# RustAudio/lewton

Measured on AMD Instinct MI355X. Metric: audio packets/sec (44.1 kHz stereo, 2048-pt long blocks), higher is better.
Workload: dtype f32; 1 GPU; BASELINE configs[1]: batches of 4096 synthetic 44.1 kHz stereo long-block (n=2048) packets per GPU = 256 streams x 16 consecutive packets, 8 batches rotated, records resident in HBM; streams_per_batch=256, channels=2, blocksize=2048, output=i16 planar, kernels=k_long, parity=unchecked (bench.py --full checks the timed batch against the oracle), parallelism=streams sharded across GPUs, no collectives

## Files before the change

lewton_amd/build.py:

```python
import os
import subprocess
import sys

HERE = os.path.dirname(os.path.abspath(__file__))
CSRC = os.path.join(HERE, "csrc")
LIBDIR = os.path.join(HERE, "_lib")
LIB = os.path.join(LIBDIR, "liblewton_amd.so")
SOURCES = ["lw_headers.cpp", "lw_entropy.cpp", "lw_dev_entropy.cpp", "lw_pool.cpp", "lw_runtime.cpp", "lw_batch.cpp", "lw_packet.cpp", "lw_fast.cpp", "lw_ring.cpp", "lw_shard.cpp", "lw_ogg.cpp", "lw_rows.cpp", "lw_rows_mix.cpp", "lw_capi.cpp", "lw_kernels.hip", "lw_kernels_long.hip", "lw_kernels_big.hip", "lw_kernels_entropy.hip", "lw_kernels_rows.hip", "lw_kernels_rows_mix.hip"]
ARCH = os.environ.get("LW_OFFLOAD_ARCH", "gfx950")
FLAGS = ["--offload-arch=" + ARCH, "-O3", "-std=c++17", "-ffp-contract=off", "-fno-fast-math", "-fPIC", "-Wall",
         "-Wno-unused-result", "-pthread"]


PER_FILE_FLAGS = {"lw_kernels_long.hip": ["-fno-slp-vectorize"]}


def hipcc():
    for c in (os.environ.get("HIPCC"), "/opt/rocm/bin/hipcc", "hipcc"):
        if c and (os.path.isabs(c) and os.path.exists(c) or not os.path.isabs(c)):
            return c
    raise RuntimeError("hipcc not found")


def needs_build():
    if not os.path.exists(LIB):
        return True
    t = os.path.getmtime(LIB)
    for root in (CSRC, os.path.join(HERE, "..", "include")):
        for f in os.listdir(root):
            if os.path.getmtime(os.path.join(root, f)) > t:
                return True
    return False


def build(force=False, verbose=False):
    if not force and not needs_build():
        return LIB
# ... 28 lines not shown
```

lewton_amd/csrc/lw_fast.hpp:

```cpp
#pragma once

#include "lw_host.hpp"
#include "lw_records.h"

#include <cstdint>
#include <vector>

#define LW_FAST_BS 11
#define LW_FAST_MAX_FLOORS 2
#define LW_FLOOR_EXACT_ADX 4096u
#define LW_FAST_WAVES 16
#define LW_FAST_MAX_ROUNDS 16

struct LwFastImage {
	uint32_t apair;
	uint32_t tw_s2;
	uint32_t tw_l0;
	uint32_t tw_l1;
	uint32_t tw_l2;
	uint32_t tw_l3;
	uint32_t tw_l4;
	uint32_t a2;
	uint32_t c4;
	uint32_t b_lo;
// ... 92 lines not shown
	LwFastImage off;
	const uint8_t *d_image;
	const LwFastItem *d_items;
	uint32_t n_items;
	const LwFastItem *d_halo_items;
	uint32_t n_halo_items;
	uint32_t n_units;
	uint32_t per_round;
	uint32_t rounds;
	uint32_t dense;
	uint32_t late_from;
	uint32_t has_tdonly;
	uint32_t split;
	uint32_t edge_mode;
	float *d_edge;
	uint32_t edge_n;
	const uint16_t *d_sid12;
	LwFastUnit units[LW_FAST_WAVES];
	float *d_halo;
	uint32_t pre_on;
	uint32_t pre[LW_FAST_WAVES];
};

#define LW_BLK_MIN_BS 8
#define LW_BLK_MAX_BS 10
#define LW_BLK_MAX_SLOTS 8
#define LW_BIG_MIN_BS 12
#define LW_BIG_MAX_BS 13
#define LW_BIG_MAX_PASSES 64u
#define LW_BLK_MAX_POSTS(L) ((L) >= 16 ? 64 : 32)

template <int L>
struct LwBlkLayout {
	static constexpr uint32_t APAIR = 0;
	static constexpr uint32_t TW_S2 = APAIR + 64u * L;
	static constexpr uint32_t TW_L0 = TW_S2 + 32u * L;
	static constexpr uint32_t TW_L1 = TW_L0 + 16u * L;
	static constexpr uint32_t TW_C2 = TW_L1 + 8u * L;
	static constexpr uint32_t TW_C3 = TW_C2 + 128u;
	static constexpr uint32_t A2 = TW_C3 + 64u;
	static constexpr uint32_t C4 = A2 + 16u;
	static constexpr uint32_t B_LO = C4 + 32u * L;
	static constexpr uint32_t B_HI = B_LO + 32u * L;
	static constexpr uint32_t WIN = B_HI + 32u * L;
	static constexpr uint32_t INV_DB = WIN + 64u * L;
	static constexpr uint32_t XSF = INV_DB + 1024u;
// ... 99 lines not shown
```

lewton_amd/csrc/lw_kernels_long.hip:

```cpp
#include <algorithm>
#include <cstddef>
#include <mutex>

#include "lw_fast.hpp"
#include "lw_kernels.hpp"
#include "lw_pcm_store.inc"

#define LW_WG (64 * LW_FAST_WAVES)
#define LW_PRIO_FLOOR 2
#define LW_PRIO_IMDCT 0
#define LW_PRIO_FINISH 3
#define LW_FLOOR_FIRST_FROM 7
#define LW_IMDCT_PRIO_LATE 12
#define LW_PRIO_PACE 0
#define LW_PRIO_READY 3
#define LW_SCR_BYTES 4096u
#define LW_PUB_BYTES 4096u
#define LW_LDS_BYTES (LWI_TOTAL + LW_FAST_WAVES * (LW_SCR_BYTES + LW_PUB_BYTES) + 3 * LW_FAST_WAVES * 4)

#include "lw_stamps.inc"

struct LwFastArgs {
	const float *residue;
	const uint16_t *floors;
	uint32_t n_items;
	uint32_t n_units;
	uint32_t per_round;
	uint32_t rounds;
	uint32_t dense;
	uint32_t late_from;
	uint32_t ch, fstride;
	LwFastUnit waves[LW_FAST_WAVES];
	const uint8_t *image;
	const LwFastItem *items;
	float *state;
	float *td;
	float *halo;
	float *edge;
	void *out;
	uint32_t state_stride, state_chan_stride;
	uint32_t edge_n;
// ... 249 lines not shown
	    "v_cndmask_b32_e64 %10, %5, -%5, %14\n\tv_cndmask_b32_e64 %11, %7, -%7, %15\n\t"
	    "v_add_f32_e32 %8, %0, %8\n\tv_add_f32_e32 %9, %2, %9\n\tv_add_f32_e32 %10, %4, %10\n\tv_add_f32_e32 %11, %6, %11\n\t"
	    "v_cndmask_b32_e64 %1, %0, %8, %16\n\tv_cndmask_b32_e64 %3, %2, %9, %17\n\t"
	    "v_cndmask_b32_e64 %5, %4, %10, %18\n\tv_cndmask_b32_e64 %7, %6, %11, %19\n\t"
	    "v_cndmask_b32_e64 %0, %8, %0, %16\n\tv_cndmask_b32_e64 %2, %9, %2, %17\n\t"
	    "v_cndmask_b32_e64 %4, %10, %4, %18\n\tv_cndmask_b32_e64 %6, %11, %6, %19"
	    : "+v"(m0), "+v"(a0), "+v"(m1), "+v"(a1), "+v"(m2), "+v"(a2), "+v"(m3), "+v"(a3), "=&v"(t0), "=&v"(t1), "=&v"(t2), "=&v"(t3),
	      "=&s"(c0), "=&s"(c1), "=&s"(c2), "=&s"(c3), "=&s"(d0), "=&s"(d1), "=&s"(d2), "=&s"(d3));
}

struct ItemRegs {
	uint32_t res_off, floor_off, out_off, src_arg;
	int32_t state_out;
	uint32_t halo_out, src_kind, flags;
	uint32_t pkt;
};

struct Pref {
	float4_t r[2][4];
	uint32_t fe[2];
};


__device__ __forceinline__ void issue_floor_loads(const LwFastArgs &F, const ItemRegs &it, const LwFastUnit &un, uint32_t lane,
		Pref &p)
{
	const uint16_t *f0 = F.floors + it.floor_off + (uint32_t)un.ch_a * F.fstride;
	p.fe[0] = lane < un.F_a ? (uint32_t)f0[lane] : 0u;
	p.fe[1] = 0u;
	if (un.ch_b >= 0) {
		const uint16_t *f1 = F.floors + it.floor_off + (uint32_t)un.ch_b * F.fstride;
		p.fe[1] = lane < un.F_b ? (uint32_t)f1[lane] : 0u;
	}
}

template <bool PAIR = false, bool NT = true>
__device__ __forceinline__ void issue_residue_loads(const LwFastArgs &F, const ItemRegs &it, const LwFastUnit &un,
		uint32_t lane, Pref &p)
{
	const float4_t *s0 = reinterpret_cast<const float4_t *>(F.residue + it.res_off + (uint32_t)un.ch_a * 1024u);
#pragma unroll
	for (int x = 0; x < 4; x++)
		p.r[0][x] = NT ? __builtin_nontemporal_load(&s0[64 * x + lane]) : s0[64 * x + lane];
	if (PAIR || un.ch_b >= 0) {
		const float4_t *s1 = reinterpret_cast<const float4_t *>(F.residue + it.res_off + (uint32_t)un.ch_b * 1024u);
#pragma unroll
		for (int x = 0; x < 4; x++)
			p.r[1][x] = NT ? __builtin_nontemporal_load(&s1[64 * x + lane]) : s1[64 * x + lane];
	}
}

template <bool NT = true>
__device__ __forceinline__ void issue_loads(const LwFastArgs &F, const ItemRegs &it, const LwFastUnit &un, uint32_t lane, Pref &p)
{
	issue_residue_loads<false, NT>(F, it, un, lane, p);
	issue_floor_loads(F, it, un, lane, p);
}

struct PreRegs {
	float4_t t[2][4];
};

__device__ __forceinline__ void issue_pre_loads(const LwFastArgs &F, const ItemRegs &it, uint32_t prog, uint32_t lane, PreRegs &q)
{
#pragma unroll
	for (int k = 0; k < 2; k++) {
		const uint32_t c = (prog >> (8 * k)) & 0xffu;
		if (c != LW_PRE_NO_CH) {
			const float4_t *s = reinterpret_cast<const float4_t *>(F.residue + it.res_off + c * 1024u);
#pragma unroll
			for (int x = 0; x < 4; x++)
				q.t[k][x] = s[64 * x + lane];
		} else {
#pragma unroll
			for (int x = 0; x < 4; x++)
				asm volatile("" : "=v"(q.t[k][x]));
		}
	}
}

#define LW_FLOOR_W0 2097153.0f
#define LW_FLOOR_MASK 0x7fcu
__device__ __forceinline__ bool floor_table(const LwFastArgs &F, const char *img, char *sc, uint32_t lane, uint32_t e,
		uint32_t fslot, uint32_t Fp)
{
	const bool unused = __builtin_amdgcn_readfirstlane(e) == LW_FLOOR_UNUSED;
// ... 473 lines not shown
#pragma nounroll
		for (uint32_t i = 0; i < n; i++) {
			switch ((prog >> (16u + 4u * i)) & 0xfu) {
			case 0x1: couple_quad(v0, v1); break;
			case 0x2: couple_quad(v0, v2); break;
			case 0x3: couple_quad(v0, v3); break;
			case 0x4: couple_quad(v1, v0); break;
			case 0x6: couple_quad(v1, v2); break;
			case 0x7: couple_quad(v1, v3); break;
			case 0x8: couple_quad(v2, v0); break;
			case 0x9: couple_quad(v2, v1); break;
			case 0xb: couple_quad(v2, v3); break;
			case 0xc: couple_quad(v3, v0); break;
			case 0xd: couple_quad(v3, v1); break;
			case 0xe: couple_quad(v3, v2); break;
			default: break;
			}
		}
		pf.r[0][x] = v0;
		pf.r[1][x] = v1;
	}
}

template <int NCH, bool SPLIT = false>
__device__ __forceinline__ void spectrum_fused(const LwFastArgs &F, const char *img, char *sc, uint32_t lane,
		const LwFastUnit &un, Pref &pf)
{
	__builtin_amdgcn_s_setprio(LW_PRIO_FLOOR);
	const bool unused0 = floor_table(F, img, sc, lane, pf.fe[0], un.floor_a, un.F_a);
	bool unused1 = false;
	if (NCH == 2)
		unused1 = floor_table(F, img, sc + 1024, lane, pf.fe[1], un.floor_b, un.F_b);
	lds_fence();
	if (NCH == 2 && un.coupled)
		decouple_pair(pf);
	if (SPLIT && NCH == 1 && un.coupled >= LW_UNIT_SPLIT_MAG) {
		if (un.coupled == LW_UNIT_SPLIT_ANG) {
#pragma unroll
			for (int x = 0; x < 4; x++) {
				const float4_t t = pf.r[0][x];
				pf.r[0][x] = pf.r[1][x];
				pf.r[1][x] = t;
			}
			decouple_pair(pf);
#pragma unroll
			for (int x = 0; x < 4; x++)
				pf.r[0][x] = pf.r[1][x];
		} else {
			decouple_pair(pf);
		}
	}
// ... 331 lines not shown
	}
}

typedef uint32_t u32x8_t __attribute__((ext_vector_type(8)));

__device__ __forceinline__ ItemRegs load_item(const LwFastItem *items, uint32_t idx)
{
	const LwFastItem *p = items + __builtin_amdgcn_readfirstlane(idx);
	u32x8_t v;
	asm volatile("s_load_dwordx8 %0, %1, 0x0\n\ts_waitcnt lgkmcnt(0)" : "=s"(v) : "s"(p) : "memory");
	ItemRegs it;
	it.res_off = v[0];
	it.floor_off = v[1];
	it.out_off = v[2];
	it.src_arg = v[3];
	it.state_out = (int32_t)v[4];
	it.halo_out = v[5];
	it.src_kind = v[6] & 0xffu;
	it.flags = (v[6] >> 16) & 0xffu;
	it.pkt = v[7];
	return it;
}

__device__ __forceinline__ void dense_offsets(const LwFastArgs &F, uint32_t item, ItemRegs &it)
{
	it.res_off = item * F.ch * 1024u;
	it.floor_off = item * F.ch * F.fstride;
}

#define LW_CNT_BASE (LWI_TOTAL + LW_FAST_WAVES * (LW_SCR_BYTES + LW_PUB_BYTES))
#define LW_CNT_PUB(w) (LW_CNT_BASE + 4u * (w))
#define LW_CNT_ACK(w) (LW_CNT_BASE + 4u * (LW_FAST_WAVES + (w)))
#define LW_CNT_LANDED(w) (LW_CNT_BASE + 4u * (2 * LW_FAST_WAVES + (w)))

__device__ __forceinline__ uint32_t lds_load_u32(uint32_t byte_addr)
{
	uint32_t v;
	asm volatile("ds_read_b32 %0, %1\n\ts_waitcnt lgkmcnt(0)" : "=v"(v) : "v"(byte_addr) : "memory");
	return v;
}

__device__ __forceinline__ void lds_store_u32(uint32_t byte_addr, uint32_t v)
{
	asm volatile("ds_write_b32 %0, %1" ::"v"(byte_addr), "v"(v) : "memory");
}

__device__ __forceinline__ void lds_wait_ge(uint32_t byte_addr, uint32_t need)
{
	while (__builtin_amdgcn_readfirstlane(lds_load_u32(byte_addr)) < need)
		__builtin_amdgcn_s_sleep(1);
}

template <int FMT, bool RIGHT_ONLY, bool TD = false, bool EDGE = false, bool SPLIT = false, bool PRE = false>
__global__ void __launch_bounds__(LW_WG) k_long(LwFastArgs F)
{
	constexpr bool MIXF = false, mix_drop_flags = false;
	uint32_t *const edge_flags = nullptr;
#include "lw_long_body.inc"
}

#define LW_SHORT_SPLIT_BELOW 1024u

template <int L>
struct LwBlkLds {
	static constexpr uint32_t SLOTS = 64u / L;
	static constexpr uint32_t POSTS = LW_BLK_MAX_POSTS(L);
	static constexpr uint32_t PT = POSTS / L;
};

template <int L, bool ONE = false>
struct LwBlkWave {
	static constexpr uint32_t SLOTS = 64u / L, POSTS = LW_BLK_MAX_POSTS(L), CH = ONE ? 1u : 2u;
	static constexpr uint32_t SCR = 0;
	static constexpr uint32_t PUB = 4096u;
	static constexpr uint32_t PUB_PASS = SLOTS * CH * 2u * L * 16u;
	static constexpr uint32_t REC = PUB + (ONE ? 1u : 2u) * PUB_PASS;
	static constexpr uint32_t TAB = REC + SLOTS * CH * POSTS * 2u;
	static constexpr uint32_t BYTES = TAB + SLOTS * CH * POSTS * 16u;
};
static_assert(LwBlkWave<8>::PUB_PASS == 4096u && LwBlkWave<32>::PUB_PASS == 4096u, "right parts of one pass: 4 KB");

// ... 304 lines not shown
	const uint32_t i = wave - (LW_FAST_WAVES - LW_MIX_SHORT_WAVES);
	const uint32_t wid = blockIdx.x * LW_MIX_SHORT_WAVES + i;
	if (wid >= F.n_waves)
		return;
	char *const smem_all = smem_dyn + LW_MIX_IMG_OFF;
	char *const smem = smem_dyn + LWI_TOTAL + (i < 2u ? 0u : LW_FAST_WAVES * LW_SCR_BYTES) + LW_MIX_LONG_WAVES * LW_SCR_BYTES +
		(i & 1u) * LwBlkWave<L, true>::BYTES;
	constexpr bool STAGE = false;
	if (__builtin_amdgcn_readfirstlane((uint32_t)F.units[wid % F.n_units].slot) == 0u) {
		constexpr int ONLY = 0;
#include "lw_short_body.inc"
	} else {
		constexpr int ONLY = 1;
#include "lw_short_body.inc"
	}
}

template <int FMT>
__global__ void __launch_bounds__(LW_WG) k_mix(LwFastArgs F, LwShortArgs FS, LwMixArgs M)
{
	constexpr bool RIGHT_ONLY = false, TD = false, EDGE = true, SPLIT = true, MIXF = true, PRE = false;
	uint32_t *const edge_flags = M.flags;
	const bool mix_drop_flags = M.drop_flags != 0;
#define LW_LONG_BODY_AFTER_STAGE                                                  \
	if (wave >= LW_FAST_WAVES - LW_MIX_SHORT_WAVES) {                            \
		mix_short_role<FMT>(FS, M, smem, wave, lane_id);                          \
		return;                                                                   \
	}
	static_assert(LwBlkLayout<8>::TOTAL / 16u <= 256u + 64u, "one 16-byte row per thread of four waves, a second one for the first 64");
#define LW_LONG_BODY_STAGE_LOAD                                                                       \
	const bool s_on = t >= 512u, s_two = s_on && t - 512u < LwBlkLayout<8>::TOTAL / 16u - 256u;       \
	const uint4 *s_src = reinterpret_cast<const uint4 *>(FS.image) + (s_on ? t - 512u : 0u);          \
	uint4 s_v0 = make_uint4(0, 0, 0, 0), s_v1 = s_v0;                                                 \
	if (s_on)                                                                                         \
		s_v0 = s_src[0];                                                                              \
	if (s_two)                                                                                        \
		s_v1 = s_src[256];
#define LW_LONG_BODY_STAGE_STORE                                                                      \
	uint4 *s_dst = reinterpret_cast<uint4 *>(smem + LW_MIX_IMG_OFF) + (s_on ? t - 512u : 0u);         \
	if (s_on)                                                                                         \
		s_dst[0] = s_v0;                                                                              \
	if (s_two)                                                                                        \
		s_dst[256] = s_v1;
#include "lw_long_body.inc"
#undef LW_LONG_BODY_AFTER_STAGE
#undef LW_LONG_BODY_STAGE_LOAD
#undef LW_LONG_BODY_STAGE_STORE
}

template <int L>
static hipError_t launch_short(LwShortArgs &F, int fmt, hipStream_t st)
{
	const dim3 grid(F.n_waves), block(64);
	return lw_with_out_fmt(fmt, [&](auto f) { return lw_launch_k(k_short<f.value, L>, grid, block, 0, st, F); });
}

static void short_prepare(const LwDevTables &T, const LwBatchDev &B, const LwShortLaunch &L, void *out, LwShortArgs &F)
{
	F.residue = B.residue;
	F.floors = B.floors;
	F.slots = L.d_slots;
	F.image = L.d_image;
	F.state = B.state;
	F.td = B.td;
	F.edge = L.d_edge;
	F.out = out;
	F.ch = T.ch;
// ... 29 lines not shown
	if (L.lanes == 16)
		return launch_short<16>(F, fmt, st);
	if (L.lanes == 32)
		return launch_short<32>(F, fmt, st);
	return hipErrorInvalidValue;
}

static hipError_t long_prepare(const LwDevTables &T, const LwBatchDev &B, const LwFastLaunch &L, void *out, hipStream_t st, LwFastArgs &F,
		uint32_t &grid)
{
	F.image = L.d_image;
	F.residue = B.residue;
	F.floors = B.floors;
	F.state = B.state;
	F.td = B.td;
	F.ch = T.ch;
	F.fstride = T.fstride;
	F.state_stride = T.state_stride;
	F.state_chan_stride = T.state_chan_stride;
	F.n_units = L.n_units;
	F.halo = L.d_halo;
	F.edge = L.d_edge;
	F.out = out;
	const size_t lds = LW_LDS_BYTES + LW_STAMP_LDS_EXTRA;
	for (uint32_t w = 0; w < LW_FAST_WAVES; w++) {
		F.waves[w] = L.units[w % L.n_units];
		F.waves[w].slot = (uint8_t)(w / L.n_units);
		F.pre[w] = L.pre_on ? L.pre[w % L.n_units] : 0u;
	}
	F.late_from = 0xFFFFFFFFu;
	static LwPerDeviceOnce once;
	const hipError_t attr_err = once.run([] {
		const void *fns[] = {(const void *)k_long<LW_OUT_I16_PLANAR, false>, (const void *)k_long<LW_OUT_I16_INTERLEAVED, false>,
			(const void *)k_long<LW_OUT_I16_ITL_STEREO, false>, (const void *)k_long<LW_OUT_F32_PLANAR, false>,
			(const void *)k_long<LW_OUT_I16_PLANAR, true>, (const void *)k_long<LW_OUT_I16_PLANAR, false, true>,
			(const void *)k_long<LW_OUT_I16_INTERLEAVED, false, true>, (const void *)k_long<LW_OUT_I16_ITL_STEREO, false, true>,
			(const void *)k_long<LW_OUT_F32_PLANAR, false, true>, (const void *)k_long<LW_OUT_I16_PLANAR, false, false, true>,
			(const void *)k_long<LW_OUT_I16_INTERLEAVED, false, false, true>, (const void *)k_long<LW_OUT_F32_PLANAR, false, false, true>,
			(const void *)k_long<LW_OUT_I16_PLANAR, true, false, false, true>,
			(const void *)k_long<LW_OUT_I16_PLANAR, false, false, false, true>, (const void *)k_long<LW_OUT_I16_INTERLEAVED, false, false, false, true>,
			(const void *)k_long<LW_OUT_F32_PLANAR, false, false, false, true>, (const void *)k_long<LW_OUT_I16_PLANAR, false, false, true, true>,
			(const void *)k_long<LW_OUT_I16_INTERLEAVED, false, false, true, true>, (const void *)k_long<LW_OUT_F32_PLANAR, false, false, true, true>,
			(const void *)k_mix<LW_OUT_I16_PLANAR>, (const void *)k_mix<LW_OUT_I16_INTERLEAVED>, (const void *)k_mix<LW_OUT_F32_PLANAR>,
			(const void *)k_long<LW_OUT_I16_PLANAR, true, false, false, false, true>,
			(const void *)k_long<LW_OUT_I16_PLANAR, false, false, false, false, true>, (const void *)k_long<LW_OUT_I16_INTERLEAVED, false, false, false, false, true>,
			(const void *)k_long<LW_OUT_F32_PLANAR, false, false, false, false, true>,
			(const void *)k_long<LW_OUT_I16_PLANAR, false, true, false, false, true>, (const void *)k_long<LW_OUT_I16_INTERLEAVED, false, true, false, false, true>,
// ... 2 lines not shown
			(const void *)k_long<LW_OUT_F32_PLANAR, false, false, true, false, true>,
			(const void *)k_long<LW_OUT_F32_ITL_STEREO, false>, (const void *)k_long<LW_OUT_F32_ITL_STEREO, false, true>,
			(const void *)k_long<LW_OUT_F32_INTERLEAVED, false>, (const void *)k_long<LW_OUT_F32_INTERLEAVED, false, true>,
			(const void *)k_long<LW_OUT_F32_INTERLEAVED, false, false, true>, (const void *)k_long<LW_OUT_F32_INTERLEAVED, false, false, false, true>,
			(const void *)k_long<LW_OUT_F32_INTERLEAVED, false, false, true, true>,
			(const void *)k_long<LW_OUT_F32_INTERLEAVED, false, false, false, false, true>,
			(const void *)k_long<LW_OUT_F32_INTERLEAVED, false, true, false, false, true>,
			(const void *)k_long<LW_OUT_F32_INTERLEAVED, false, false, true, false, true>, (const void *)k_mix<LW_OUT_F32_INTERLEAVED>};
		for (const void *f : fns) {
			const hipError_t e = hipFuncSetAttribute(f, hipFuncAttributeMaxDynamicSharedMemorySize, 160 * 1024);
			if (e != hipSuccess)
				return e;
		}
		return hipSuccess;
	});
	if (attr_err != hipSuccess)
		return attr_err;
	if (L.n_halo_items) {
		F.items = L.d_halo_items;
		F.n_items = L.n_halo_items;
		F.per_round = 1;
		F.rounds = 1;
		const hipError_t e = L.pre_on
			? lw_launch_k(k_long<LW_OUT_I16_PLANAR, true, false, false, false, true>, dim3(L.n_halo_items), dim3(LW_WG), lds, st, F)
			: L.split
			? lw_launch_k(k_long<LW_OUT_I16_PLANAR, true, false, false, true>, dim3(L.n_halo_items), dim3(LW_WG), lds, st, F)
			: lw_launch_k(k_long<LW_OUT_I16_PLANAR, true>, dim3(L.n_halo_items), dim3(LW_WG), lds, st, F);
		if (e != hipSuccess)
			return e;
	}
	grid = 0;
	if (L.n_items) {
		F.items = L.d_items;
		F.n_items = L.n_items;
		F.per_round = L.per_round;
		F.rounds = L.rounds;
		F.dense = L.dense;
		const uint32_t chunk = L.per_round * L.rounds;
		grid = (L.n_items + chunk - 1) / chunk;
		F.late_from = L.late_from;
	}
	return hipSuccess;
}

template <int FMT>
static hipError_t launch_long_main(const LwFastLaunch &L, LwFastArgs &F, uint32_t grid, size_t lds, hipStream_t st)
{
	constexpr int FP = lw_out_unit_free(FMT);
	if (L.pre_on) {
		if (L.edge_mode)
			return lw_launch_k(k_long<FP, false, false, true, false, true>, dim3(grid), dim3(LW_WG), lds, st, F);
		if (L.has_tdonly)
			return lw_launch_k(k_long<FP, false, true, false, false, true>, dim3(grid), dim3(LW_WG), lds, st, F);
		return lw_launch_k(k_long<FP, false, false, false, false, true>, dim3(grid), dim3(LW_WG), lds, st, F);
	}
	if (L.split && !L.has_tdonly) {
		if (L.edge_mode)
			return lw_launch_k(k_long<FP, false, false, true, true>, dim3(grid), dim3(LW_WG), lds, st, F);
		return lw_launch_k(k_long<FP, false, false, false, true>, dim3(grid), dim3(LW_WG), lds, st, F);
	}
	if (L.edge_mode)
		return lw_launch_k(k_long<FP, false, false, true>, dim3(grid), dim3(LW_WG), lds, st, F);
	if (L.has_tdonly)
		return lw_launch_k(k_long<FMT, false, true>, dim3(grid), dim3(LW_WG), lds, st, F);
	return lw_launch_k(k_long<FMT, false, false>, dim3(grid), dim3(LW_WG), lds, st, F);
}

hipError_t lw_launch_long(const LwDevTables &T, const LwBatchDev &B, const LwFastLaunch &L, void *out, int fmt, hipStream_t st)
{
	LwFastArgs F{};
	uint32_t grid = 0;
	const hipError_t pe = long_prepare(T, B, L, out, st, F, grid);
	if (pe != hipSuccess || !L.n_items)
		return pe;
	const size_t lds = LW_LDS_BYTES + LW_STAMP_LDS_EXTRA;
	const bool unit2 = F.ch == 2 && L.n_units == 1 && L.units[0].ch_b >= 0;
	return lw_with_out_fmt(fmt, [&](auto f) {
		constexpr int FS = f.value == LW_OUT_I16_INTERLEAVED ? LW_OUT_I16_ITL_STEREO
			: f.value == LW_OUT_F32_INTERLEAVED ? LW_OUT_F32_ITL_STEREO : f.value;
		return unit2 ? launch_long_main<FS>(L, F, grid, lds, st) : launch_long_main<f.value>(L, F, grid, lds, st);
	});
}

bool lw_mix_applicable(const LwFastLaunch &LL, const LwShortLaunch &LS, int n_cus)
{
	if (!LL.n_items || !LL.split || !LL.edge_mode || LL.has_tdonly || LL.rounds != 1 || !LS.n_tasks || LS.lanes != 8 || LS.passes > 1)
		return false;
	if ((size_t)LS.n_tasks * LS.n_units > LW_SHORT_SPLIT_BELOW || 2 * LS.n_units > LW_FAST_WAVES)
		return false;
	for (uint32_t u = 0; u < LS.n_units; u++)
		if (LS.units[u].ch_b < 0)
			return false;
	if (LL.per_round * LL.n_units > LW_MIX_LONG_WAVES)
		return false;
	const uint32_t chunk = LL.per_round * LL.rounds;
	const size_t n_wg = (LL.n_items + chunk - 1) / chunk;
	return n_wg <= (size_t)std::max(1, n_cus) && (size_t)LS.n_tasks * LS.n_units * 2 <= n_wg * LW_MIX_SHORT_WAVES;
}
// ... 81 lines not shown
```

lewton_amd/csrc/lw_long_body.inc:

```
	extern __shared__ __attribute__((aligned(16))) char smem[];
	const uint32_t lane_id = threadIdx.x & 63u;
	const uint32_t wave = __builtin_amdgcn_readfirstlane(threadIdx.x >> 6);
	LW_STAMP_DECL;
	LW_STAMP(0);
	const uint32_t n_units = F.n_units, per_round = F.per_round, rounds = F.rounds;
	LwFastUnit un;
#if defined(__HIP_DEVICE_COMPILE__)
	typedef const unsigned long long __attribute__((address_space(4))) *ka_ptr;
	const unsigned long long unit_word = ((ka_ptr)__builtin_amdgcn_kernarg_segment_ptr())[offsetof(LwFastArgs, waves) / 8 + wave];
#else
	const unsigned long long unit_word = 0;
#endif
	asm volatile("" ::"s"(F.residue), "s"(F.floors), "s"(F.n_items), "s"(n_units), "s"(per_round), "s"(rounds), "s"(F.dense),
			"s"(F.late_from), "s"(F.ch), "s"(F.fstride), "s"(F.image), "s"(unit_word));
	__builtin_memcpy(&un, &unit_word, 8);
	const uint32_t slot = un.slot, uidx = wave - slot * n_units;
	const bool active = slot < per_round;
	const uint32_t item0 = blockIdx.x * per_round * rounds + slot;
	const bool two = !SPLIT && un.ch_b >= 0;
	const int chn[2] = {un.ch_a, two ? un.ch_b : un.ch_a};
	const uint32_t pre_prog = PRE ? __builtin_amdgcn_readfirstlane(F.pre[wave]) : 0u;
	PreRegs pq;
#define LW_PRE_WAVES 2
	const bool late = !RIGHT_ONLY && wave >= (F.late_from > LW_PRE_WAVES ? F.late_from : (uint32_t)LW_PRE_WAVES);

	ItemRegs it{};
	Pref pf{};
	bool valid = active && item0 < F.n_items;
	if (valid) {
		if (F.dense)
			dense_offsets(F, item0, it);
		else
			it = load_item(F.items, item0);
	}
	static_assert(LWI_TOTAL / 16 == 2 * (LW_WG - 256), "image staging: 12 waves x 2 x 16 bytes per thread");
	static_assert(LW_FLOOR_FIRST_FROM >= 4, "floor-first waves request their floor records after staging the image");
	const bool floor_first = !PRE && late && two && F.late_from < LW_FAST_WAVES && wave >= LW_FLOOR_FIRST_FROM;
	if (wave < 4) {
		if (valid && !late)
			{
				issue_loads<!PRE>(F, it, un, lane_id, pf);
				if (PRE)
					issue_pre_loads(F, it, pre_prog, lane_id, pq);
			}
	} else {
		const uint32_t t = threadIdx.x - 256u;
		const uint4 *src = reinterpret_cast<const uint4 *>(F.image) + t;
		uint4 *dst = reinterpret_cast<uint4 *>(smem) + t;
		const uint4 v0 = src[0], v1 = src[LW_WG - 256];
#ifdef LW_LONG_BODY_STAGE_LOAD
		LW_LONG_BODY_STAGE_LOAD
#endif
		if (t < 3 * LW_FAST_WAVES)
			lds_store_u32(LW_CNT_BASE + 4u * t, 0u);
		dst[0] = v0;
		dst[LW_WG - 256] = v1;
#ifdef LW_LONG_BODY_STAGE_STORE
		LW_LONG_BODY_STAGE_STORE
#endif
		lds_fence();
		if (valid && !late)
			{
				issue_loads<!PRE>(F, it, un, lane_id, pf);
				if (PRE)
					issue_pre_loads(F, it, pre_prog, lane_id, pq);
			}
		if (valid && floor_first)
			issue_floor_loads(F, it, un, lane_id, pf);
	}
	__syncthreads();
#ifdef LW_LONG_BODY_AFTER_STAGE
	LW_LONG_BODY_AFTER_STAGE
#endif
	const char *img = smem;
	LW_STAMP(2);
	char *sc = smem + LWI_TOTAL + wave * LW_SCR_BYTES;
	char *pub0 = smem + LWI_TOTAL + LW_FAST_WAVES * LW_SCR_BYTES;
	char *pub = pub0 + wave * LW_PUB_BYTES;
#define LW_PACE_VMCNT 63
	const bool paced = !RIGHT_ONLY && F.late_from < LW_FAST_WAVES;
	uint32_t lane0 = lane_id;
	asm volatile("" : "+v"(lane0));
	if (valid && floor_first) {
		float4_t fl[2][4];
		floor_phase<2>(F, img, sc, lane0, un, pf.fe, fl);
		LW_STAMP(1);
		__builtin_amdgcn_s_setprio(LW_PRIO_PACE);
		lds_wait_ge(LW_CNT_LANDED(wave - F.late_from), 1u);
		issue_residue_loads<true, !PRE>(F, it, un, lane_id, pf);
		if (PRE)
			issue_pre_loads(F, it, pre_prog, lane_id, pq);
		LW_STAMP(15);
		if (wave + F.late_from < LW_FAST_WAVES) {
			asm volatile("s_waitcnt vmcnt(%0)" ::"n"(LW_PACE_VMCNT) : "memory");
			lds_store_u32(LW_CNT_LANDED(wave), 1u);
		}
		if (F.dense)
			it = load_item(F.items, item0);
		__builtin_amdgcn_s_setprio(LW_PRIO_READY);
		LW_STAMP_W(3);
		if (PRE)
			apply_pre(pre_prog, pf, pq);
		spectrum_ready(un, pf, fl);
		__builtin_amdgcn_s_setprio(0);
		LW_STAMP(4);
	} else {
		if (paced) {
			__builtin_amdgcn_s_setprio(LW_PRIO_PACE);
			if (late) {
				lds_wait_ge(LW_CNT_LANDED(wave - F.late_from), 1u);
				if (valid)
					{
				issue_loads<!PRE>(F, it, un, lane_id, pf);
				if (PRE)
					issue_pre_loads(F, it, pre_prog, lane_id, pq);
			}
			}
			LW_STAMP(15);
			if (wave + F.late_from < LW_FAST_WAVES) {
				asm volatile("s_waitcnt vmcnt(%0)" ::"n"(LW_PACE_VMCNT) : "memory");
				lds_store_u32(LW_CNT_LANDED(wave), 1u);
			}
			__builtin_amdgcn_s_setprio(0);
		}
		if (valid && F.dense)
			it = load_item(F.items, item0);
		LW_STAMP_W(3);
		if (valid) {
			if (PRE)
				apply_pre(pre_prog, pf, pq);
			if (two)
				spectrum_fused<2>(F, img, sc, lane0, un, pf);
			else
				spectrum_fused<1, SPLIT>(F, img, sc, lane0, un, pf);
		}
		LW_STAMP(4);
	}
	uint32_t n_pub_used = 0;
	uint32_t n_got = 0;
	const uint32_t wprev = slot != 0 ? wave - n_units : (per_round - 1) * n_units + uidx;

	for (uint32_t j = 0; j < rounds; j++) {
		uint32_t lane = lane_id;
		asm volatile("" : "+v"(lane));
		float2_t R[2][2][4];
		const uint32_t item_n = item0 + (j + 1) * per_round;
		const bool valid_n = active && j + 1 < rounds && item_n < F.n_items;
		ItemRegs itn{};
		if (valid_n && !F.dense)
			itn = load_item(F.items, item_n);
		if (valid) {
			if (two)
				long_imdct<2, MIXF ? 1 : 0>(F, img, sc, lane, pf, R);
			else
				long_imdct<1, MIXF ? 1 : 0>(F, img, sc, lane, pf, R);
			if (j == 0)
				LW_STAMP(8);
		}
		if (valid) {
			if (RIGHT_ONLY) {
#pragma unroll
				for (int c = 0; c < 2; c++)
					if (c == 0 || two) {
						float *dst = F.halo + ((size_t)it.halo_out * F.ch + chn[c]) * 512u;
						*reinterpret_cast<float4_t *>(dst + 4u * lane) = LW_PB_LO0(c);
						*reinterpret_cast<float4_t *>(dst + 508u - 4u * lane) = LW_PB_LO1(c);
					}
			} else {
				__builtin_amdgcn_s_setprio(LW_PRIO_FINISH);
				const bool edge_l = EDGE && (it.flags & LW_IF_EDGE_L), edge_r = EDGE && (it.flags & LW_IF_EDGE_R);
				const uint32_t e_ls = edge_l ? 448u : 0u, e_m = EDGE ? (edge_r ? 1472u : 1024u) - e_ls : 1024u;
				if (MIXF && (edge_l || edge_r)) {
#pragma unroll
// ... 153 lines not shown
			if (F.dense) {
				dense_offsets(F, item_n, itn);
				issue_loads<!PRE>(F, itn, un, lane, pf);
				if (PRE)
					issue_pre_loads(F, itn, pre_prog, lane, pq);
				itn = load_item(F.items, item_n);
			} else {
				issue_loads<!PRE>(F, itn, un, lane, pf);
				if (PRE)
					issue_pre_loads(F, itn, pre_prog, lane, pq);
			}
			if (PRE)
				apply_pre(pre_prog, pf, pq);
			if (two)
				spectrum_fused<2>(F, img, sc, lane, un, pf);
			else
				spectrum_fused<1, SPLIT>(F, img, sc, lane, un, pf);
		}
		it = itn;
		valid = valid_n;
	}
	LW_STAMP_W(11);
	LW_STAMP_FLUSH;
```

lewton_amd/csrc/lw_stamps.inc:

```
#ifdef LW_STAMPS
__device__ unsigned long long *g_lw_stamps = nullptr;
extern "C" int lw_debug_set_stamp_buffer(void *dptr)
{
	return (int)hipMemcpyToSymbol(HIP_SYMBOL(g_lw_stamps), &dptr, sizeof(dptr));
}
#define LW_STAMP_LDS_EXTRA 2048u
#define LW_STAMP_BASE_ (LW_LDS_BYTES)
typedef __attribute__((address_space(3))) unsigned long long *lw_stamp_lds_ptr;
#define LW_STAMP_DECL                                                                                         \
	const uint32_t st_wave_ = __builtin_amdgcn_readfirstlane(threadIdx.x >> 6);                               \
	if ((threadIdx.x & 63u) < 16u)                                                                            \
		*reinterpret_cast<lw_stamp_lds_ptr>((uintptr_t)(LW_STAMP_BASE_ + st_wave_ * 128u + (threadIdx.x & 63u) * 8u)) = 0ull
#define LW_STAMP(i)                                                                                           \
	do {                                                                                                      \
		const unsigned long long t_ = __builtin_amdgcn_s_memtime();                                           \
		*reinterpret_cast<lw_stamp_lds_ptr>((uintptr_t)(LW_STAMP_BASE_ + st_wave_ * 128u + (i) * 8u)) = t_;   \
	} while (0)
#define LW_STAMP_W(i)                                                                                         \
	do {                                                                                                      \
		asm volatile("s_waitcnt vmcnt(0)" ::: "memory");                                                      \
		LW_STAMP(i);                                                                                          \
	} while (0)
#define LW_STAMP_FLUSH                                                                                        \
	do {                                                                                                      \
		unsigned long long *b_ = g_lw_stamps;                                                                 \
		if (b_ && (threadIdx.x & 63u) < 16u)                                                                  \
			b_[((size_t)blockIdx.x * LW_FAST_WAVES + st_wave_) * 16 + (threadIdx.x & 63u)] =                  \
				*reinterpret_cast<lw_stamp_lds_ptr>((uintptr_t)(LW_STAMP_BASE_ + st_wave_ * 128u + (threadIdx.x & 63u) * 8u)); \
	} while (0)
#else
#define LW_STAMP_LDS_EXTRA 0u
#define LW_STAMP_DECL
#define LW_STAMP(i)
#define LW_STAMP_W(i)
#define LW_STAMP_FLUSH
#endif
```

Measured before the change: 255.9 million packets/s.

## Preload hot kernel arguments into SGPRs and issue early loads in k_long

Passes the hot k_long fields (residue/floors/image pointers, counts, a packed word of unit/round/late/channel fields, and the first two wave unit descriptors) as leading scalar kernel arguments, and enables kernarg preloading so they arrive in SGPRs before the first instruction. Image-staging waves start their global image loads before any other setup, and the first two waves in dense mode issue their residue/floor loads immediately from the preloaded unit words. It also raises the priority of the fused spectrum phase and adds an optional floor gate counter, which is disabled by default because LW_GATE_NEED is 0. The intent is to shorten kernel prologue latency, at the cost of more launch-argument plumbing, a 16-byte LDS increase, and reliance on a compiler flag for preloading.

```diff
diff --git a/lewton_amd/build.py b/lewton_amd/build.py
--- a/lewton_amd/build.py
+++ b/lewton_amd/build.py
@@ -12,7 +12,7 @@
          "-Wno-unused-result", "-pthread"]
 
 
-PER_FILE_FLAGS = {"lw_kernels_long.hip": ["-fno-slp-vectorize"]}
+PER_FILE_FLAGS = {"lw_kernels_long.hip": ["-fno-slp-vectorize", "-mllvm", "-amdgpu-kernarg-preload-count=14"]}
 
 
 def hipcc():
diff --git a/lewton_amd/csrc/lw_fast.hpp b/lewton_amd/csrc/lw_fast.hpp
--- a/lewton_amd/csrc/lw_fast.hpp
+++ b/lewton_amd/csrc/lw_fast.hpp
@@ -138,6 +138,32 @@
 	uint32_t pre[LW_FAST_WAVES];
 };
 
+#define LW_LATE_UNPACED 0xFFFFFFFFu
+#define LW_LW_LATE_UNPACED_CODE 31u
+struct LwLongWord {
+	uint32_t n_units, per_round, dense, late_from, ch;
+};
+
+constexpr bool lw_long_word_pack(const LwLongWord &v, uint32_t *word)
+{
+	if (v.n_units < 1u || v.n_units > LW_FAST_WAVES || v.per_round < 1u || v.per_round > LW_FAST_WAVES || v.dense > 1u || v.ch < 1u ||
+			v.ch > 255u)
+		return false;
+	if (v.late_from != LW_LATE_UNPACED && (v.late_from < 1u || v.late_from > LW_FAST_WAVES))
+		return false;
+	const uint32_t late = v.late_from == LW_LATE_UNPACED ? LW_LW_LATE_UNPACED_CODE : v.late_from;
+	*word = v.n_units | v.per_round << 5 | v.dense << 10 | late << 11 | v.ch << 16;
+	return true;
+}
+
+constexpr LwLongWord lw_long_word_unpack(uint32_t word)
+{
+	const uint32_t late = (word >> 11) & 31u;
+	return LwLongWord{word & 31u, (word >> 5) & 31u, (word >> 10) & 1u, late == LW_LW_LATE_UNPACED_CODE ? LW_LATE_UNPACED : late,
+		(word >> 16) & 255u};
+}
+static_assert(LW_FAST_WAVES < LW_LW_LATE_UNPACED_CODE, "the launch word's 5-bit fields hold every wave count and the unpaced code");
+
 #define LW_BLK_MIN_BS 8
 #define LW_BLK_MAX_BS 10
 #define LW_BLK_MAX_SLOTS 8
diff --git a/lewton_amd/csrc/lw_kernels_long.hip b/lewton_amd/csrc/lw_kernels_long.hip
--- a/lewton_amd/csrc/lw_kernels_long.hip
+++ b/lewton_amd/csrc/lw_kernels_long.hip
@@ -8,15 +8,21 @@
 
 #define LW_WG (64 * LW_FAST_WAVES)
 #define LW_PRIO_FLOOR 2
+#ifndef LW_PRIO_FUSED
+#define LW_PRIO_FUSED 3
+#endif
 #define LW_PRIO_IMDCT 0
 #define LW_PRIO_FINISH 3
+#ifndef LW_FLOOR_FIRST_FROM
 #define LW_FLOOR_FIRST_FROM 7
+#endif
 #define LW_IMDCT_PRIO_LATE 12
 #define LW_PRIO_PACE 0
 #define LW_PRIO_READY 3
 #define LW_SCR_BYTES 4096u
 #define LW_PUB_BYTES 4096u
 #define LW_LDS_BYTES (LWI_TOTAL + LW_FAST_WAVES * (LW_SCR_BYTES + LW_PUB_BYTES) + 3 * LW_FAST_WAVES * 4)
+#define LW_LONG_LDS_BYTES (LW_LDS_BYTES + 16u)
 
 #include "lw_stamps.inc"
 
@@ -312,7 +318,8 @@
 };
 
 
-__device__ __forceinline__ void issue_floor_loads(const LwFastArgs &F, const ItemRegs &it, const LwFastUnit &un, uint32_t lane,
+template <class ARGS>
+__device__ __forceinline__ void issue_floor_loads(const ARGS &F, const ItemRegs &it, const LwFastUnit &un, uint32_t lane,
 		Pref &p)
 {
 	const uint16_t *f0 = F.floors + it.floor_off + (uint32_t)un.ch_a * F.fstride;
@@ -324,8 +331,8 @@
 	}
 }
 
-template <bool PAIR = false, bool NT = true>
-__device__ __forceinline__ void issue_residue_loads(const LwFastArgs &F, const ItemRegs &it, const LwFastUnit &un,
+template <bool PAIR = false, bool NT = true, class ARGS>
+__device__ __forceinline__ void issue_residue_loads(const ARGS &F, const ItemRegs &it, const LwFastUnit &un,
 		uint32_t lane, Pref &p)
 {
 	const float4_t *s0 = reinterpret_cast<const float4_t *>(F.residue + it.res_off + (uint32_t)un.ch_a * 1024u);
@@ -340,8 +347,8 @@
 	}
 }
 
-template <bool NT = true>
-__device__ __forceinline__ void issue_loads(const LwFastArgs &F, const ItemRegs &it, const LwFastUnit &un, uint32_t lane, Pref &p)
+template <bool NT = true, class ARGS>
+__device__ __forceinline__ void issue_loads(const ARGS &F, const ItemRegs &it, const LwFastUnit &un, uint32_t lane, Pref &p)
 {
 	issue_residue_loads<false, NT>(F, it, un, lane, p);
 	issue_floor_loads(F, it, un, lane, p);
@@ -351,7 +358,8 @@
 	float4_t t[2][4];
 };
 
-__device__ __forceinline__ void issue_pre_loads(const LwFastArgs &F, const ItemRegs &it, uint32_t prog, uint32_t lane, PreRegs &q)
+template <class ARGS>
+__device__ __forceinline__ void issue_pre_loads(const ARGS &F, const ItemRegs &it, uint32_t prog, uint32_t lane, PreRegs &q)
 {
 #pragma unroll
 	for (int k = 0; k < 2; k++) {
@@ -871,11 +879,11 @@
 	}
 }
 
-template <int NCH, bool SPLIT = false>
+template <int NCH, bool SPLIT = false, int PRIO = LW_PRIO_FLOOR>
 __device__ __forceinline__ void spectrum_fused(const LwFastArgs &F, const char *img, char *sc, uint32_t lane,
 		const LwFastUnit &un, Pref &pf)
 {
-	__builtin_amdgcn_s_setprio(LW_PRIO_FLOOR);
+	__builtin_amdgcn_s_setprio(PRIO);
 	const bool unused0 = floor_table(F, img, sc, lane, pf.fe[0], un.floor_a, un.F_a);
 	bool unused1 = false;
 	if (NCH == 2)
@@ -1253,7 +1261,8 @@
 	return it;
 }
 
-__device__ __forceinline__ void dense_offsets(const LwFastArgs &F, uint32_t item, ItemRegs &it)
+template <class ARGS>
+__device__ __forceinline__ void dense_offsets(const ARGS &F, uint32_t item, ItemRegs &it)
 {
 	it.res_off = item * F.ch * 1024u;
 	it.floor_off = item * F.ch * F.fstride;
@@ -1263,6 +1272,7 @@
 #define LW_CNT_PUB(w) (LW_CNT_BASE + 4u * (w))
 #define LW_CNT_ACK(w) (LW_CNT_BASE + 4u * (LW_FAST_WAVES + (w)))
 #define LW_CNT_LANDED(w) (LW_CNT_BASE + 4u * (2 * LW_FAST_WAVES + (w)))
+#define LW_CNT_SPEC (LW_CNT_BASE + 4u * (3 * LW_FAST_WAVES))
 
 __device__ __forceinline__ uint32_t lds_load_u32(uint32_t byte_addr)
 {
@@ -1282,12 +1292,80 @@
 		__builtin_amdgcn_s_sleep(1);
 }
 
+__device__ __forceinline__ void lds_add_u32(uint32_t byte_addr, uint32_t v)
+{
+	asm volatile("ds_add_u32 %0, %1" ::"v"(byte_addr), "v"(v) : "memory");
+}
+
+#define LW_GATE_POLLS 128u
+#ifndef LW_GATE_NEED
+#define LW_GATE_NEED(w) 0u
+#endif
+__device__ __forceinline__ bool floor_gate(uint32_t need, uint32_t landed_addr)
+{
+#pragma nounroll
+	for (uint32_t i = 0; i < LW_GATE_POLLS; i++) {
+		uint32_t c, l;
+		asm volatile("ds_read_b32 %0, %2\n\tds_read_b32 %1, %3\n\ts_waitcnt lgkmcnt(0)"
+				: "=&v"(c), "=&v"(l)
+				: "v"(LW_CNT_SPEC), "v"(landed_addr)
+				: "memory");
+		if (__builtin_amdgcn_readfirstlane(l) != 0u)
+			return true;
+		if (__builtin_amdgcn_readfirstlane(c) >= need)
+			return false;
+		__builtin_amdgcn_s_sleep(2);
+	}
+	return false;
+}
+
+struct LwLongHot {
+	const float *residue;
+	const uint16_t *floors;
+	const uint8_t *image;
+	uint32_t n_items, n_units, per_round, rounds, dense, late_from, ch, fstride;
+};
+#define LW_LONG_PRELOAD_DWORDS 14
+
 template <int FMT, bool RIGHT_ONLY, bool TD = false, bool EDGE = false, bool SPLIT = false, bool PRE = false>
-__global__ void __launch_bounds__(LW_WG) k_long(LwFastArgs F)
+__global__ void __launch_bounds__(LW_WG) k_long(const float *h_residue, const uint16_t *h_floors, const uint8_t *h_image, uint32_t h_n_items,
+		uint32_t h_word, uint32_t h_rounds, uint32_t h_fstride, unsigned long long h_unit0, unsigned long long h_unit1, LwFastArgs F)
 {
 	constexpr bool MIXF = false, mix_drop_flags = false;
 	uint32_t *const edge_flags = nullptr;
+	const LwLongWord hw = lw_long_word_unpack(h_word);
+	const LwLongHot H{h_residue, h_floors, h_image, h_n_items, hw.n_units, hw.per_round, h_rounds, hw.dense, hw.late_from, hw.ch, h_fstride};
+#define LW_LONG_BODY_HOT_UNITS
 #include "lw_long_body.inc"
+#undef LW_LONG_BODY_HOT_UNITS
+}
+
+template <class K>
+static hipError_t launch_k_long(K kernel, dim3 grid, size_t lds, hipStream_t st, LwFastArgs &F)
+{
+	uint32_t word = 0;
+	if (!lw_long_word_pack(LwLongWord{F.n_units, F.per_round, F.dense, F.late_from, F.ch}, &word))
+		return hipErrorInvalidValue;
+	unsigned long long u0, u1;
+	static_assert(offsetof(LwFastArgs, waves) % 8 == 0 && sizeof(LwFastUnit) == 8, "unit words");
+	__builtin_memcpy(&u0, &F.waves[0], 8);
+	__builtin_memcpy(&u1, &F.waves[1], 8);
+	return lw_launch_k(kernel, grid, dim3(LW_WG), lds, st, F.residue, F.floors, F.image, F.n_items, word, F.rounds, F.fstride, u0, u1, F);
+}
+
+extern "C" int lw_debug_long_word_pack(uint32_t n_units, uint32_t per_round, uint32_t dense, uint32_t late_from, uint32_t ch, uint32_t *word)
+{
+	return lw_long_word_pack(LwLongWord{n_units, per_round, dense, late_from, ch}, word) ? 0 : -1;
+}
+
+extern "C" void lw_debug_long_word_unpack(uint32_t word, uint32_t *out5)
+{
+	const LwLongWord v = lw_long_word_unpack(word);
+	out5[0] = v.n_units;
+	out5[1] = v.per_round;
+	out5[2] = v.dense;
+	out5[3] = v.late_from;
+	out5[4] = v.ch;
 }
 
 #define LW_SHORT_SPLIT_BELOW 1024u
@@ -1638,6 +1716,7 @@
 	constexpr bool RIGHT_ONLY = false, TD = false, EDGE = true, SPLIT = true, MIXF = true, PRE = false;
 	uint32_t *const edge_flags = M.flags;
 	const bool mix_drop_flags = M.drop_flags != 0;
+#define H F
 #define LW_LONG_BODY_AFTER_STAGE                                                  \
 	if (wave >= LW_FAST_WAVES - LW_MIX_SHORT_WAVES) {                            \
 		mix_short_role<FMT>(FS, M, smem, wave, lane_id);                          \
@@ -1659,6 +1738,7 @@
 	if (s_two)                                                                                        \
 		s_dst[256] = s_v1;
 #include "lw_long_body.inc"
+#undef H
 #undef LW_LONG_BODY_AFTER_STAGE
 #undef LW_LONG_BODY_STAGE_LOAD
 #undef LW_LONG_BODY_STAGE_STORE
@@ -1734,7 +1814,7 @@
 	F.halo = L.d_halo;
 	F.edge = L.d_edge;
 	F.out = out;
-	const size_t lds = LW_LDS_BYTES + LW_STAMP_LDS_EXTRA;
+	const size_t lds = LW_LONG_LDS_BYTES + LW_STAMP_LDS_EXTRA;
 	for (uint32_t w = 0; w < LW_FAST_WAVES; w++) {
 		F.waves[w] = L.units[w % L.n_units];
 		F.waves[w].slot = (uint8_t)(w / L.n_units);
@@ -1783,10 +1863,10 @@
 		F.per_round = 1;
 		F.rounds = 1;
 		const hipError_t e = L.pre_on
-			? lw_launch_k(k_long<LW_OUT_I16_PLANAR, true, false, false, false, true>, dim3(L.n_halo_items), dim3(LW_WG), lds, st, F)
+			? launch_k_long(k_long<LW_OUT_I16_PLANAR, true, false, false, false, true>, dim3(L.n_halo_items), lds, st, F)
 			: L.split
-			? lw_launch_k(k_long<LW_OUT_I16_PLANAR, true, false, false, true>, dim3(L.n_halo_items), dim3(LW_WG), lds, st, F)
-			: lw_launch_k(k_long<LW_OUT_I16_PLANAR, true>, dim3(L.n_halo_items), dim3(LW_WG), lds, st, F);
+			? launch_k_long(k_long<LW_OUT_I16_PLANAR, true, false, false, true>, dim3(L.n_halo_items), lds, st, F)
+			: launch_k_long(k_long<LW_OUT_I16_PLANAR, true>, dim3(L.n_halo_items), lds, st, F);
 		if (e != hipSuccess)
 			return e;
 	}
@@ -1810,21 +1890,21 @@
 	constexpr int FP = lw_out_unit_free(FMT);
 	if (L.pre_on) {
 		if (L.edge_mode)
-			return lw_launch_k(k_long<FP, false, false, true, false, true>, dim3(grid), dim3(LW_WG), lds, st, F);
+			return launch_k_long(k_long<FP, false, false, true, false, true>, dim3(grid), lds, st, F);
 		if (L.has_tdonly)
-			return lw_launch_k(k_long<FP, false, true, false, false, true>, dim3(grid), dim3(LW_WG), lds, st, F);
-		return lw_launch_k(k_long<FP, false, false, false, false, true>, dim3(grid), dim3(LW_WG), lds, st, F);
+			return launch_k_long(k_long<FP, false, true, false, false, true>, dim3(grid), lds, st, F);
+		return launch_k_long(k_long<FP, false, false, false, false, true>, dim3(grid), lds, st, F);
 	}
 	if (L.split && !L.has_tdonly) {
 		if (L.edge_mode)
-			return lw_launch_k(k_long<FP, false, false, true, true>, dim3(grid), dim3(LW_WG), lds, st, F);
-		return lw_launch_k(k_long<FP, false, false, false, true>, dim3(grid), dim3(LW_WG), lds, st, F);
+			return launch_k_long(k_long<FP, false, false, true, true>, dim3(grid), lds, st, F);
+		return launch_k_long(k_long<FP, false, false, false, true>, dim3(grid), lds, st, F);
 	}
 	if (L.edge_mode)
-		return lw_launch_k(k_long<FP, false, false, true>, dim3(grid), dim3(LW_WG), lds, st, F);
+		return launch_k_long(k_long<FP, false, false, true>, dim3(grid), lds, st, F);
 	if (L.has_tdonly)
-		return lw_launch_k(k_long<FMT, false, true>, dim3(grid), dim3(LW_WG), lds, st, F);
-	return lw_launch_k(k_long<FMT, false, false>, dim3(grid), dim3(LW_WG), lds, st, F);
+		return launch_k_long(k_long<FMT, false, true>, dim3(grid), lds, st, F);
+	return launch_k_long(k_long<FMT, false, false>, dim3(grid), lds, st, F);
 }
 
 hipError_t lw_launch_long(const LwDevTables &T, const LwBatchDev &B, const LwFastLaunch &L, void *out, int fmt, hipStream_t st)
@@ -1834,7 +1914,7 @@
 	const hipError_t pe = long_prepare(T, B, L, out, st, F, grid);
 	if (pe != hipSuccess || !L.n_items)
 		return pe;
-	const size_t lds = LW_LDS_BYTES + LW_STAMP_LDS_EXTRA;
+	const size_t lds = LW_LONG_LDS_BYTES + LW_STAMP_LDS_EXTRA;
 	const bool unit2 = F.ch == 2 && L.n_units == 1 && L.units[0].ch_b >= 0;
 	return lw_with_out_fmt(fmt, [&](auto f) {
 		constexpr int FS = f.value == LW_OUT_I16_INTERLEAVED ? LW_OUT_I16_ITL_STEREO
diff --git a/lewton_amd/csrc/lw_long_body.inc b/lewton_amd/csrc/lw_long_body.inc
--- a/lewton_amd/csrc/lw_long_body.inc
+++ b/lewton_amd/csrc/lw_long_body.inc
@@ -1,19 +1,61 @@
 	extern __shared__ __attribute__((aligned(16))) char smem[];
+	constexpr bool GATE = !MIXF && !RIGHT_ONLY && !PRE && !SPLIT;
 	const uint32_t lane_id = threadIdx.x & 63u;
 	const uint32_t wave = __builtin_amdgcn_readfirstlane(threadIdx.x >> 6);
 	LW_STAMP_DECL;
 	LW_STAMP(0);
-	const uint32_t n_units = F.n_units, per_round = F.per_round, rounds = F.rounds;
+	LW_STAMP_SIMD(13);
+	const uint32_t n_units = H.n_units, per_round = H.per_round, rounds = H.rounds;
+#ifdef LW_LONG_BODY_HOT_UNITS
+#define LW_LONG_BODY_ROUNDS F.rounds
+#else
+#define LW_LONG_BODY_ROUNDS rounds
+#endif
+#define LW_PRE_WAVES 2
+#ifdef LW_LONG_BODY_HOT_UNITS
+	ItemRegs it{};
+	Pref pf{};
+	bool early = false;
+	uint4 stage_v0 = make_uint4(0, 0, 0, 0), stage_v1 = stage_v0;
+	if (wave >= 4u) {
+		const uint4 *src = reinterpret_cast<const uint4 *>(H.image) + (threadIdx.x - 256u);
+		stage_v0 = src[0];
+		stage_v1 = src[LW_WG - 256];
+	} else if (!PRE && wave < LW_PRE_WAVES && H.dense) {
+		LwFastUnit u0;
+		const unsigned long long w0 = wave ? h_unit1 : h_unit0;
+		__builtin_memcpy(&u0, &w0, 8);
+		const uint32_t item_e = blockIdx.x * per_round * rounds + u0.slot;
+		if (u0.slot < per_round && item_e < H.n_items) {
+			dense_offsets(H, item_e, it);
+			issue_loads<true>(H, it, u0, lane_id, pf);
+			early = true;
+		}
+	}
+#else
+	constexpr bool early = false;
+#endif
 	LwFastUnit un;
 #if defined(__HIP_DEVICE_COMPILE__)
 	typedef const unsigned long long __attribute__((address_space(4))) *ka_ptr;
+#ifdef LW_LONG_BODY_HOT_UNITS
+	constexpr uint32_t ka_waves = (LW_LONG_PRELOAD_DWORDS * 4u + offsetof(LwFastArgs, waves)) / 8u;
+	static_assert(LW_LONG_PRELOAD_DWORDS % 2 == 0, "F follows the leading parameters without padding");
+	unsigned long long unit_word = wave ? h_unit1 : h_unit0;
+	if (wave >= 2u)
+		unit_word = ((ka_ptr)__builtin_amdgcn_kernarg_segment_ptr())[ka_waves + wave];
+#else
 	const unsigned long long unit_word = ((ka_ptr)__builtin_amdgcn_kernarg_segment_ptr())[offsetof(LwFastArgs, waves) / 8 + wave];
+#endif
 #else
 	const unsigned long long unit_word = 0;
 #endif
+#ifndef LW_LONG_BODY_HOT_UNITS
 	asm volatile("" ::"s"(F.residue), "s"(F.floors), "s"(F.n_items), "s"(n_units), "s"(per_round), "s"(rounds), "s"(F.dense),
 			"s"(F.late_from), "s"(F.ch), "s"(F.fstride), "s"(F.image), "s"(unit_word));
+#endif
 	__builtin_memcpy(&un, &unit_word, 8);
+	LW_STAMP_ARGS(5, un);
 	const uint32_t slot = un.slot, uidx = wave - slot * n_units;
 	const bool active = slot < per_round;
 	const uint32_t item0 = blockIdx.x * per_round * rounds + slot;
@@ -21,37 +63,42 @@
 	const int chn[2] = {un.ch_a, two ? un.ch_b : un.ch_a};
 	const uint32_t pre_prog = PRE ? __builtin_amdgcn_readfirstlane(F.pre[wave]) : 0u;
 	PreRegs pq;
-#define LW_PRE_WAVES 2
-	const bool late = !RIGHT_ONLY && wave >= (F.late_from > LW_PRE_WAVES ? F.late_from : (uint32_t)LW_PRE_WAVES);
+	const bool late = !RIGHT_ONLY && wave >= (H.late_from > LW_PRE_WAVES ? H.late_from : (uint32_t)LW_PRE_WAVES);
 
+#ifndef LW_LONG_BODY_HOT_UNITS
 	ItemRegs it{};
 	Pref pf{};
-	bool valid = active && item0 < F.n_items;
+#endif
+	bool valid = active && item0 < H.n_items;
 	if (valid) {
-		if (F.dense)
-			dense_offsets(F, item0, it);
+		if (H.dense)
+			dense_offsets(H, item0, it);
 		else
 			it = load_item(F.items, item0);
 	}
 	static_assert(LWI_TOTAL / 16 == 2 * (LW_WG - 256), "image staging: 12 waves x 2 x 16 bytes per thread");
 	static_assert(LW_FLOOR_FIRST_FROM >= 4, "floor-first waves request their floor records after staging the image");
-	const bool floor_first = !PRE && late && two && F.late_from < LW_FAST_WAVES && wave >= LW_FLOOR_FIRST_FROM;
+	const bool floor_first = !PRE && late && two && H.late_from < LW_FAST_WAVES && wave >= LW_FLOOR_FIRST_FROM;
 	if (wave < 4) {
-		if (valid && !late)
+		if (valid && !late && !early)
 			{
-				issue_loads<!PRE>(F, it, un, lane_id, pf);
+				issue_loads<!PRE>(H, it, un, lane_id, pf);
 				if (PRE)
-					issue_pre_loads(F, it, pre_prog, lane_id, pq);
+					issue_pre_loads(H, it, pre_prog, lane_id, pq);
 			}
 	} else {
 		const uint32_t t = threadIdx.x - 256u;
-		const uint4 *src = reinterpret_cast<const uint4 *>(F.image) + t;
 		uint4 *dst = reinterpret_cast<uint4 *>(smem) + t;
+#ifdef LW_LONG_BODY_HOT_UNITS
+		const uint4 v0 = stage_v0, v1 = stage_v1;
+#else
+		const uint4 *src = reinterpret_cast<const uint4 *>(H.image) + t;
 		const uint4 v0 = src[0], v1 = src[LW_WG - 256];
+#endif
 #ifdef LW_LONG_BODY_STAGE_LOAD
 		LW_LONG_BODY_STAGE_LOAD
 #endif
-		if (t < 3 * LW_FAST_WAVES)
+		if (t < 3 * LW_FAST_WAVES + (GATE ? 1 : 0))
 			lds_store_u32(LW_CNT_BASE + 4u * t, 0u);
 		dst[0] = v0;
 		dst[LW_WG - 256] = v1;
@@ -61,12 +108,12 @@
 		lds_fence();
 		if (valid && !late)
 			{
-				issue_loads<!PRE>(F, it, un, lane_id, pf);
+				issue_loads<!PRE>(H, it, un, lane_id, pf);
 				if (PRE)
-					issue_pre_loads(F, it, pre_prog, lane_id, pq);
+					issue_pre_loads(H, it, pre_prog, lane_id, pq);
 			}
 		if (valid && floor_first)
-			issue_floor_loads(F, it, un, lane_id, pf);
+			issue_floor_loads(H, it, un, lane_id, pf);
 	}
 	__syncthreads();
 #ifdef LW_LONG_BODY_AFTER_STAGE
@@ -78,24 +125,35 @@
 	char *pub0 = smem + LWI_TOTAL + LW_FAST_WAVES * LW_SCR_BYTES;
 	char *pub = pub0 + wave * LW_PUB_BYTES;
 #define LW_PACE_VMCNT 63
-	const bool paced = !RIGHT_ONLY && F.late_from < LW_FAST_WAVES;
+	const bool paced = !RIGHT_ONLY && H.late_from < LW_FAST_WAVES;
 	uint32_t lane0 = lane_id;
 	asm volatile("" : "+v"(lane0));
-	if (valid && floor_first) {
+	const bool floor_now = valid && floor_first;
+	if (floor_now)
+		LW_STAMP_W(6);
+	if (GATE && floor_now) {
+		const uint32_t need = LW_GATE_NEED(wave);
+		if (need) {
+			__builtin_amdgcn_s_setprio(LW_PRIO_PACE);
+			floor_gate(need, LW_CNT_LANDED(wave - H.late_from));
+		}
+	}
+	if (floor_now) {
 		float4_t fl[2][4];
+		LW_STAMP(7);
 		floor_phase<2>(F, img, sc, lane0, un, pf.fe, fl);
 		LW_STAMP(1);
 		__builtin_amdgcn_s_setprio(LW_PRIO_PACE);
-		lds_wait_ge(LW_CNT_LANDED(wave - F.late_from), 1u);
-		issue_residue_loads<true, !PRE>(F, it, un, lane_id, pf);
+		lds_wait_ge(LW_CNT_LANDED(wave - H.late_from), 1u);
+		issue_residue_loads<true, !PRE>(H, it, un, lane_id, pf);
 		if (PRE)
-			issue_pre_loads(F, it, pre_prog, lane_id, pq);
+			issue_pre_loads(H, it, pre_prog, lane_id, pq);
 		LW_STAMP(15);
-		if (wave + F.late_from < LW_FAST_WAVES) {
+		if (wave + H.late_from < LW_FAST_WAVES) {
 			asm volatile("s_waitcnt vmcnt(%0)" ::"n"(LW_PACE_VMCNT) : "memory");
 			lds_store_u32(LW_CNT_LANDED(wave), 1u);
 		}
-		if (F.dense)
+		if (H.dense)
 			it = load_item(F.items, item0);
 		__builtin_amdgcn_s_setprio(LW_PRIO_READY);
 		LW_STAMP_W(3);
@@ -108,32 +166,34 @@
 		if (paced) {
 			__builtin_amdgcn_s_setprio(LW_PRIO_PACE);
 			if (late) {
-				lds_wait_ge(LW_CNT_LANDED(wave - F.late_from), 1u);
+				lds_wait_ge(LW_CNT_LANDED(wave - H.late_from), 1u);
 				if (valid)
 					{
-				issue_loads<!PRE>(F, it, un, lane_id, pf);
+				issue_loads<!PRE>(H, it, un, lane_id, pf);
 				if (PRE)
-					issue_pre_loads(F, it, pre_prog, lane_id, pq);
+					issue_pre_loads(H, it, pre_prog, lane_id, pq);
 			}
 			}
 			LW_STAMP(15);
-			if (wave + F.late_from < LW_FAST_WAVES) {
+			if (wave + H.late_from < LW_FAST_WAVES) {
 				asm volatile("s_waitcnt vmcnt(%0)" ::"n"(LW_PACE_VMCNT) : "memory");
 				lds_store_u32(LW_CNT_LANDED(wave), 1u);
 			}
 			__builtin_amdgcn_s_setprio(0);
 		}
-		if (valid && F.dense)
+		if (valid && H.dense)
 			it = load_item(F.items, item0);
 		LW_STAMP_W(3);
 		if (valid) {
 			if (PRE)
 				apply_pre(pre_prog, pf, pq);
 			if (two)
-				spectrum_fused<2>(F, img, sc, lane0, un, pf);
+				spectrum_fused<2, false, MIXF ? LW_PRIO_FLOOR : LW_PRIO_FUSED>(F, img, sc, lane0, un, pf);
 			else
-				spectrum_fused<1, SPLIT>(F, img, sc, lane0, un, pf);
-		}
+				spectrum_fused<1, SPLIT, MIXF ? LW_PRIO_FLOOR : LW_PRIO_FUSED>(F, img, sc, lane0, un, pf);
+		}
+		if (GATE && wave < LW_FLOOR_FIRST_FROM && lane_id == 0u)
+			lds_add_u32(LW_CNT_SPEC, 1u);
 		LW_STAMP(4);
 	}
 	uint32_t n_pub_used = 0;
@@ -145,10 +205,12 @@
 		asm volatile("" : "+v"(lane));
 		float2_t R[2][2][4];
 		const uint32_t item_n = item0 + (j + 1) * per_round;
-		const bool valid_n = active && j + 1 < rounds && item_n < F.n_items;
+		const bool valid_n = active && j + 1 < LW_LONG_BODY_ROUNDS && item_n < F.n_items;
 		ItemRegs itn{};
 		if (valid_n && !F.dense)
 			itn = load_item(F.items, item_n);
+		if (j == 0)
+			LW_STAMP(12);
 		if (valid) {
 			if (two)
 				long_imdct<2, MIXF ? 1 : 0>(F, img, sc, lane, pf, R);
@@ -348,3 +410,4 @@
 	}
 	LW_STAMP_W(11);
 	LW_STAMP_FLUSH;
+#undef LW_LONG_BODY_ROUNDS
diff --git a/lewton_amd/csrc/lw_stamps.inc b/lewton_amd/csrc/lw_stamps.inc
--- a/lewton_amd/csrc/lw_stamps.inc
+++ b/lewton_amd/csrc/lw_stamps.inc
@@ -5,7 +5,7 @@
 	return (int)hipMemcpyToSymbol(HIP_SYMBOL(g_lw_stamps), &dptr, sizeof(dptr));
 }
 #define LW_STAMP_LDS_EXTRA 2048u
-#define LW_STAMP_BASE_ (LW_LDS_BYTES)
+#define LW_STAMP_BASE_ (LW_LONG_LDS_BYTES)
 typedef __attribute__((address_space(3))) unsigned long long *lw_stamp_lds_ptr;
 #define LW_STAMP_DECL                                                                                         \
 	const uint32_t st_wave_ = __builtin_amdgcn_readfirstlane(threadIdx.x >> 6);                               \
@@ -21,6 +21,16 @@
 		asm volatile("s_waitcnt vmcnt(0)" ::: "memory");                                                      \
 		LW_STAMP(i);                                                                                          \
 	} while (0)
+#define LW_STAMP_SIMD(i)                                                                                      \
+	do {                                                                                                      \
+		const unsigned long long t_ = 1ull + (unsigned long long)__builtin_amdgcn_s_getreg(4 | (4 << 6) | (1 << 11)); \
+		*reinterpret_cast<lw_stamp_lds_ptr>((uintptr_t)(LW_STAMP_BASE_ + st_wave_ * 128u + (i) * 8u)) = t_;   \
+	} while (0)
+#define LW_STAMP_ARGS(i, un)                                                                                  \
+	do {                                                                                                      \
+		asm volatile("" ::"s"(H.residue), "s"(H.floors), "s"(H.image), "s"(H.n_items), "s"(H.fstride), "s"((uint32_t)(un).slot)); \
+		LW_STAMP(i);                                                                                          \
+	} while (0)
 #define LW_STAMP_FLUSH                                                                                        \
 	do {                                                                                                      \
 		unsigned long long *b_ = g_lw_stamps;                                                                 \
@@ -33,5 +43,7 @@
 #define LW_STAMP_DECL
 #define LW_STAMP(i)
 #define LW_STAMP_W(i)
+#define LW_STAMP_SIMD(i)
+#define LW_STAMP_ARGS(i, un)
 #define LW_STAMP_FLUSH
 #endif
```

Measured after the change: 253.6 million packets/s. Within noise of the previous version (-0.9%).
